# ppwwyyxx/speaker-recognition

Hardware: AMD Instinct MI355X
Metric: frames/sec scored (MFCC+GMM) (higher is better)
Workload: dtype f32

## Files before the change

speaker-recognition_amd/csrc/abi.cpp:

```cpp
#include "../../include/pygmm_hip.h"

#include "batch.hpp"
#include "common.hpp"
#include "fork_proxy.hpp"
#include "gmm_full.hpp"
#include "gmm_model.hpp"
#include "mfcc.hpp"
#include "mfcc_plan.hpp"
#include "score.hpp"
#include "silence_plan.hpp"
#include "topc_plan.hpp"
#include "bw_plan.hpp"
#include "jfa_plan.hpp"
#include "map_plan.hpp"

#include <algorithm>
#include <cmath>
#include <cstring>
#include <fstream>
#include <limits>
#include <sstream>

namespace sr {
void burn_reference_rand(int count);
// ... 1132 lines not shown
    ltsd_compute(*pcm, winsize, order, noise_amp, ltsd_out, win_offsets_out);
    return 0;
    SR_CATCH(-1)
}

int sr_set_option(const char *key, long value) {
    SR_TRY
    if (!key) fail("null key");
    const std::string k(key);
    if (k == "score_frames_per_lane") {
        if (value != 0 && value != 1 && value != 2 && value != 4) fail("frames per lane must be 0/1/2/4");
        score_options().frames_per_lane = (int)value;
    } else if (k == "score_model_groups") {
        score_options().model_groups = (int)value;
    } else if (k == "score_packed") {
        score_options().packed = (int)value;
    } else if (k == "score_engine") {
        if (value < 0 || value > 6 || value == 2)
            fail("score_engine must be 0 (auto), 1 (vector ALU), 3 (split-bf16 matrix cores), 4 (split-bf16, shared-sigma form), "
                 "5 (split-fp16 matrix cores) or 6 (split-fp16, shared-sigma form); 2 was the fp32 matrix-core engine, removed in round 5 "
                 "(never selected: 1.45-1.8x slower than split-bf16 at the same accuracy)");
        score_options().engine = (int)value;
    } else if (k == "score_h2s_shape") {
        if (value < 0 || value > 5)
            fail("score_h2s_shape must be 0 (automatic), 1 (4-wave workgroups), 2 (12-wave workgroups), 3 (12 waves, image loop pipelined inside the wave), "
                 "4 (4 waves on one tile, the block's models split between them) or 5 (as 3, on the flat image where 3 takes the compact one)");
        score_options().h2s_shape = (int)value;
    } else if (k == "flush_list_cap") {
        if (value < 0) fail("flush_list_cap must be >= 0");
        score_options().flush_list_cap = (int)value;
    } else if (k == "score_h2s_pack_tails") {
        if (value != 0 && value != 1) fail("score_h2s_pack_tails must be 0 or 1");
        score_options().h2s_pack_tails = (int)value;
    } else if (k == "score_h2s_force_exc") {
        score_options().h2s_force_exc = value != 0;
    } else if (k == "score_split_shape") {
        if (value != 0 && value != 1 && value != 8 && value != 12 && value != 16)
            fail("score_split_shape must be 0 (automatic), 1 (4-wave workgroups) or 8 / 12 / 16 (waves of the wide, pipelined form)");
        score_options().split_shape = (int)value;
    } else if (k == "score_mfma_ft") {
        if (value < 0 || value > 4) fail("score_mfma_ft must be 0..4");
        score_options().mfma_ft = (int)value;
    } else if (k == "flush_order") {
        if (value != 1 && value != 2)
            fail("flush_order must be 2 (partial products as the reference DSO's compiler forms them: even / odd dimensions) or "
                 "1 (the source's order, gmm.cc:192-195)");
        flush_order_option() = (int)value;
    } else if (k == "kmeans_assign_engine") {
        if (value != 0 && value != 1) fail("kmeans_assign_engine must be 0 (fast full search, exact pass for what it cannot decide) or 1 (exact pass only)");
// ... 219 lines not shown
```

speaker-recognition_amd/csrc/gmm_score_h2_shared.hip:

```cpp
#include "lse.hpp"
#include "score.hpp"
#include "wave_ops.hpp"

#include <algorithm>
#include <cstdint>
#include <type_traits>

namespace sr {

typedef float f32x16 __attribute__((ext_vector_type(16)));
typedef _Float16 f16x8 __attribute__((ext_vector_type(8)));
typedef unsigned u32x4 __attribute__((ext_vector_type(4)));

constexpr int H2S_ROUNDS_PER_LAUNCH = 12;
constexpr float H2S_SUM_LO = 7.8886090522101181e-31f;
constexpr float H2S_SUM_HI = 1.2676506002282294e+30f;
constexpr float H2S_LOG2E = 1.4426950408889634f;

template <int KN, int KM, int COLS>
__device__ __forceinline__ void h2s_chain_regs(f32x16 (&acc)[COLS], const f32x16 (&init)[COLS], const uint4 (&fr)[KM],
                                               const f16x8 (&b)[COLS][KN]) {
#pragma unroll
    for (int ks = 0; ks < KN; ks++)
#pragma unroll
// ... 518 lines not shown
    else if constexpr (NX == 1) H2P_SLOT_ASM(H, R, NA_, 1);     \
    else if constexpr (NX == 2) H2P_SLOT_ASM(H, R, NA_, 2);     \
    else if constexpr (NX == 3) H2P_SLOT_ASM(H, R, NA_, 3);     \
    else H2P_SLOT_ASM(H, R, NA_, 4);
#define H2P_SLOT_NA(H, R)                                \
    if constexpr (NA == 0) { H2P_SLOT_NX(H, R, 0) }      \
    else if constexpr (NA == 1) { H2P_SLOT_NX(H, R, 1) } \
    else if constexpr (NA == 2) { H2P_SLOT_NX(H, R, 2) } \
    else if constexpr (NA == 3) { H2P_SLOT_NX(H, R, 3) } \
    else { H2P_SLOT_NX(H, R, 4) }
template <int HEAD, bool READ, int NA, int NX, int W, int O>
__device__ __forceinline__ void h2p_slot(f32x16 &cur, u32x4 &fu, float &s, float &e0, float &e1, float &e2, float &e3, const f16x8 &b, const f32x16 &c,
                                         unsigned at, float p0, float p1, float p2, float p3) {
    static_assert(NA <= 4 && NX <= 4, "at most four exps per slot");
    if constexpr (HEAD == 0) {
        if constexpr (READ) { H2P_SLOT_NA(0, 1) } else { H2P_SLOT_NA(0, 0) }
    } else if constexpr (HEAD == 1) {
        if constexpr (READ) { H2P_SLOT_NA(1, 1) } else { H2P_SLOT_NA(1, 0) }
    } else {
        if constexpr (READ) { H2P_SLOT_NA(2, 1) } else { H2P_SLOT_NA(2, 0) }
    }
}

template <int KQF, int KLF, bool CPT = false>
__global__ __launch_bounds__(12 * 64, 3)
void gmm_score_h2p_kernel(const H2sArgs a) {
    constexpr int SB = SHARED_SB, WAVES = 12, G = 4, NB = 2, DMA_AT = KLF / 2;
    constexpr int KM = KQF > KLF ? KQF : KLF;
    static_assert(KQF <= KLF, "the linear half is never the shorter one");
    static_assert(!CPT || (KQF == H2C_KLF && KLF == H2C_KLF), "the compact order is built for the <8,8> chains");
    static_assert(!CPT || h2c_map_ok(H2C_MAP), "compact order");
    constexpr int NF = CPT ? H2C_MAP.nf : KM;
    constexpr int NBQ = CPT ? H2C_MAP.nb : KQF, NBL = CPT ? H2C_MAP.nb : KLF;
    constexpr int IMG_U4 = NF * 64;
    constexpr int STAGE_U4 = G * IMG_U4;
    constexpr int N_IMG = 1 + SB;
    constexpr int N_STAGES = N_IMG / G;
    static_assert(N_IMG % G == 0 && N_STAGES >= 1, "stages tile the images of a mixture tile");
    extern __shared__ uint4 h2s_bq_lds[];
    __shared__ uint4 ring[NB * STAGE_U4];

    const int tid = threadIdx.x;
    const int lane = tid & 63;
    const int wave = __builtin_amdgcn_readfirstlane(tid >> 6);
    const int col = lane & 31;
    const int hh = lane >> 5;

    constexpr int N_PIECES = STAGE_U4 / 64;
    constexpr int P_LO = N_PIECES / WAVES, P_HI = (N_PIECES + WAVES - 1) / WAVES, N_HI = N_PIECES % WAVES;
    auto stage_load = [&](int slot, const uint4 *src) {
#pragma unroll
        for (int i = 0; i < P_HI; i++) {
            const int piece = i * WAVES + wave;
            if (piece < N_PIECES)
                __builtin_amdgcn_global_load_lds(
                    (const __attribute__((address_space(1))) void *)(src + piece * 64 + lane),
                    (__attribute__((address_space(3))) void *)(ring + slot * STAGE_U4 + piece * 64), 16, 0, 0);
        }
    };
    auto wait_stages = [&](int keep) {
        if (keep <= 0 || P_HI == 0) {
// ... 26 lines not shown
        tile = a.tiles[has ? tids[0] : 0];
#pragma unroll
        for (int p = 1; p < 4; p++)
            if (p < n_seg && col >= first_col[p]) {
                my_col = col - first_col[p];
                tile = a.tiles[tids[p]];
            }
    }
    const bool valid = has && my_col < tile.count;
    const int64_t row = tile.start + (valid ? my_col : 0);
    {
        f16x8 bq[NBQ];
        h2s_build_b<NBQ>(bq, a.X + row * a.dim, a.center, a.scale, a.q_desc, hh, true, zmax);
#pragma unroll
        for (int ks = 0; ks < NBQ; ks++) h2s_bq_lds[(wave * NBQ + ks) * 64 + lane] = __builtin_bit_cast(uint4, bq[ks]);
    }
    h2s_build_b<NBL>(bl, a.X + row * a.dim, a.center, a.scale, a.l_desc, hh, false, zmax);
    const float off = a.ref_ll[row] * H2S_LOG2E;
    if (zmax >= 255.0f) atomicOr(a.oor_flag, 1);
    const float safe_ll2 = a.clamp ? fmaxf(LSE_MINLOG2 + LSE_NEAR + a.log2_k, a.band_hi * H2S_LOG2E + 1.0f) : -3.0e38f;
    const f32x16 zero1 = {0, 0, 0, 0, 0, 0, 0, 0, 0, 0, 0, 0, 0, 0, 0, 0};
    const unsigned ring_lane = (unsigned)(uintptr_t)(__attribute__((address_space(3))) void *)ring + (unsigned)lane * 16u;

    for (int blk = blk_begin; blk < blk_end; blk++) {
        const SharedBlock sb = a.blocks[blk];
        const uint4 *stream = a.params + sb.offset_u4;
        float ssum[SB + 1];
#pragma unroll
        for (int si = 0; si <= SB; si++) ssum[si] = 0.0f;
        const int n_st = (1 + sb.n_models + G - 1) / G;
        const int n_stage_total = a.n_mix_tiles * n_st;
        int ld_tile = 0, ld_st = 0;
        auto stage_load_next = [&](int slot) {
            stage_load(slot, stream + (size_t)ld_tile * (N_IMG * IMG_U4) + (size_t)ld_st * STAGE_U4);
            if (++ld_st == n_st) {
                ld_st = 0;
                ld_tile++;
            }
        };
        u32x4 fr[NF];
        auto frag_read = [&](auto U, unsigned at) {
            constexpr int u = decltype(U)::value;
            u32x4 &dst = fr[u];
            asm volatile("ds_read_b128 %0, %1 offset:%2" : "=v"(dst) : "v"(at), "n"(u * 1024));
        };

        asm volatile("s_waitcnt lgkmcnt(0)" ::: "memory");
        barrier();
        stage_load_next(0);
        if (n_stage_total > 1) stage_load_next(1);
        if (NB > 2 && n_stage_total > 2) stage_load_next(2);
        wait_stages(n_stage_total > NB - 1 ? NB - 1 : n_stage_total - 1);
        barrier();
        h2p_for<0, (CPT ? NF : KQF)>([&](auto U) { frag_read(U, ring_lane); });

        f32x16 acc[2];
        acc[0] = zero1;
#pragma unroll
        for (int r = 0; r < 16; r++) acc[1][r] = -1.0e30f;
        int S = 0, slot_cur = 0, slot_nxt = 1;
        static_assert(NB == 2 || NB == 3, "ring of two or three stages");
        f32x16 qacc = zero1;
        float e[16] = {0.0f, 0.0f, 0.0f, 0.0f};
        for (int t = 0; t < a.n_mix_tiles; t++) {
            h2p_for<0, N_IMG>([&](auto IMG) {
                constexpr int img = decltype(IMG)::value;
                constexpr int gi = img % G;
                constexpr int kn = img == 0 ? KQF : KLF;
                constexpr int kn_next = img + 1 == N_IMG ? KQF : KLF;
                constexpr bool carry = img != 1;
                constexpr int prev_model = img == 0 ? SB : img - 2;
                if (img / G >= n_st) return;
                if constexpr (gi == G - 1) {
                    wait_stages(NB > 2 && S + 2 < n_stage_total ? 1 : 0);
                    barrier();
                    if constexpr (DMA_AT == 0)
                        if (S + NB < n_stage_total) stage_load_next(slot_cur);
                }
                const unsigned next_at = ring_lane + (unsigned)((gi == G - 1 ? slot_nxt * STAGE_U4 : slot_cur * STAGE_U4 + (gi + 1) * IMG_U4) * 16);
                f32x16 &cur = img == 0 ? qacc : acc[img & 1];
                const f32x16 &prev = acc[(img & 1) ^ 1];
                constexpr int BW = KQF < 4 ? KQF : 4;
                f16x8 bqt[BW];
                auto bq_load = [&](int ks) { return __builtin_bit_cast(f16x8, h2s_bq_lds[(wave * NBQ + ks) * 64 + lane]); };
                if constexpr (img == 0) {
                    if constexpr (CPT) {
                        h2p_for<0, BW>([&](auto KS) { bqt[decltype(KS)::value] = bq_load(H2C_MAP.b_of[decltype(KS)::value]); });
                    } else {
#pragma unroll
                        for (int ks = 0; ks < BW; ks++) bqt[ks] = bq_load(ks);
                    }
                }
                constexpr bool ONE_ASM = kn >= 5;
                static_assert(!CPT || ONE_ASM, "the compact order is written for the one-statement slots");
                constexpr int sum_model = carry ? prev_model : 0;
                if constexpr (ONE_ASM) {
                    h2p_for<0, kn>([&](auto U) {
                        constexpr int u = decltype(U)::value;
                        if constexpr (gi == G - 1 && DMA_AT != 0 && u == DMA_AT)
                            if (S + NB < n_stage_total) stage_load_next(slot_cur);
                        constexpr int fa = CPT ? H2C_MAP.a_of[u] : u, bi = CPT ? H2C_MAP.b_of[u] : u;
                        constexpr bool rd = CPT ? H2C_MAP.a_last[fa] == u : (u < kn_next);
                        constexpr int younger = CPT ? h2c_younger(H2C_MAP, u) : (kn - 1 - u) + (u < kn_next ? u : kn_next);
                        static_assert(younger <= 15, "lgkmcnt is a 4-bit field");
                        constexpr int e0 = carry ? h2p_cum(kn, u - 2) : 0, e1 = carry ? h2p_cum(kn, u - 1) : 0, e2 = carry ? h2p_cum(kn, u) : 0;
                        constexpr int NA = e1 - e0, NX = e2 - e1;
                        const float p0 = prev[e1 < 16 ? e1 : 15], p1 = prev[e1 + 1 < 16 ? e1 + 1 : 15], p2 = prev[e1 + 2 < 16 ? e1 + 2 : 15],
                                    p3 = prev[e1 + 3 < 16 ? e1 + 3 : 15];
                        if constexpr (img == 0)
                        {
                            h2p_slot<u == 0 ? 0 : 2, rd, NA, NX, younger, fa * 1024>(cur, fr[fa], ssum[sum_model], e[0], e[1], e[2], e[3], bqt[u % BW],
                                                                                     qacc, next_at, p0, p1, p2, p3);
                            if constexpr (u + BW < KQF) bqt[u % BW] = bq_load(CPT ? H2C_MAP.b_of[u + BW] : u + BW);
                        }
                        else
                            h2p_slot<u == 0 ? 1 : 2, rd, NA, NX, younger, fa * 1024>(cur, fr[fa], ssum[sum_model], e[0], e[1], e[2], e[3], bl[bi], qacc,
                                                                                     next_at, p0, p1, p2, p3);
                        __builtin_amdgcn_sched_barrier(0);
                    });
                } else {
                    h2p_for<0, kn>([&](auto U) {
                        constexpr int u = decltype(U)::value;
                        if constexpr (gi == G - 1 && DMA_AT != 0 && u == DMA_AT)
                            if (S + NB < n_stage_total) stage_load_next(slot_cur);
                        constexpr int younger = (kn - 1 - u) + (u < kn_next ? u : kn_next);
                        u32x4 &fu = fr[u];
                        asm volatile("s_waitcnt lgkmcnt(%1)" : "+v"(fu) : "n"(younger));
                        if constexpr (img == 0)
                            cur = __builtin_amdgcn_mfma_f32_32x32x16_f16(__builtin_bit_cast(f16x8, fr[u]), bqt[u % BW], u == 0 ? zero1 : cur, 0, 0, 0);
                        else
                            cur = __builtin_amdgcn_mfma_f32_32x32x16_f16(__builtin_bit_cast(f16x8, fr[u]), bl[u], u == 0 ? qacc : cur, 0, 0, 0);
                        f32x16 &cpin = cur;
                        asm volatile("" : "+v"(cpin));
                        if constexpr (u < kn_next) frag_read(U, next_at);
                        if constexpr (carry) {
                            constexpr int e0 = h2p_cum(kn, u - 2), e1 = h2p_cum(kn, u - 1), e2 = h2p_cum(kn, u);
                            h2p_for<e0, e1>([&](auto R) {
                                float &sv = ssum[prev_model];
                                const float ev = e[decltype(R)::value - e0];
                                asm volatile("v_add_f32 %0, %0, %1" : "+v"(sv) : "v"(ev));
                            });
                            h2p_for<e1, e2>([&](auto R) {
                                float &ev = e[decltype(R)::value - e1];
                                const float pv = prev[decltype(R)::value];
                                asm volatile("v_exp_f32 %0, %1" : "=v"(ev) : "v"(pv));
                            });
                        }
                        __builtin_amdgcn_sched_barrier(0);
                    });
                }
                if constexpr (!CPT) h2p_for<kn, kn_next>([&](auto U) { frag_read(U, next_at); });
                if constexpr (carry) {
                    constexpr int e0 = h2p_cum(kn, kn - 2), e1 = h2p_cum(kn, kn - 1);
                    if constexpr (kn <= 1) {
#pragma unroll
                        for (int r = 0; r < 16; r++) ssum[prev_model] += __builtin_amdgcn_exp2f(prev[r]);
                    } else {
                        asm volatile("s_nop 0");
                        h2p_for<e0, e1>([&](auto R) {
                            float &sv = ssum[prev_model];
                            const float ev = e[decltype(R)::value - e0];
                            asm volatile("v_add_f32 %0, %0, %1" : "+v"(sv) : "v"(ev));
                        });
                    }
                }
                if constexpr (img == 0) {
                    asm volatile("s_nop 12");
                    h2p_for<0, 16>([&](auto R) {
                        float x = qacc[decltype(R)::value];
                        asm volatile("v_sub_f32 %0, %0, %1" : "+v"(x) : "v"(off));
                        qacc[decltype(R)::value] = x;
                    });
                    asm volatile("s_nop 1");
                }
                __builtin_amdgcn_sched_barrier(0);
                if constexpr (gi == G - 1) {
                    S++;
                    slot_cur = slot_nxt;
                    slot_nxt = slot_nxt == NB - 1 ? 0 : slot_nxt + 1;
                }
            });
        }
        asm volatile("s_nop 12");
#pragma unroll
        for (int r = 0; r < 16; r++) ssum[SB] += __builtin_amdgcn_exp2f(acc[(N_IMG - 1) & 1][r]);
        float fin[SB];
        const int last_model = n_st * G - 2;
#pragma unroll
        for (int si = 0; si < SB; si++) fin[si] = ssum[si] + (si == last_model ? ssum[SB] : 0.0f);
        {
            int tids[4], first_col[4], n_seg;
            h2p_unit(a, unit, tids, first_col, n_seg);
            if (n_seg == 1) h2s_close_block(a, sb, blk, fin, off, valid, has, tids[0], row, lane, hh, safe_ll2);
            else h2s_close_block_packed(a, sb, blk, fin, off, valid, has, tids, first_col, n_seg, row, lane, hh, safe_ll2);
        }
    }
    asm volatile("s_waitcnt lgkmcnt(0)" ::: "memory");
}

__device__ __forceinline__ int *h2s_plan_starts(const H2sArgs &a, int blk) {
    return reinterpret_cast<int *>(a.exc_list + (size_t)a.n_blocks * a.n_tiles) + (size_t)blk * (a.n_tiles + 1);
}

constexpr int H2S_PLAN_INLINE_MAX_TILES = 1024;
__device__ __forceinline__ int h2s_plan_block(const H2sArgs &a, int blk, int lane) {
    const int count = min(a.exc_count[blk], a.n_tiles);
    int *starts = h2s_plan_starts(a, blk);
    const int2 *list = a.exc_list + (size_t)blk * a.n_tiles;
    int n_items = 0, fill = 32;
    for (int base = 0; base < count; base += 64) {
        const int pop = base + lane < count ? __builtin_popcount((unsigned)list[base + lane].y) : 0;
        const int n = min(64, count - base);
        for (int i = 0; i < n; i++) {
            const int p = __builtin_amdgcn_readlane(pop, i);
            if (fill + p > 32) {
                if (lane == 0) starts[n_items] = base + i;
                n_items++;
// ... 163 lines not shown
        for (int o = 32; o > 0; o >>= 1) max_pop = max(max_pop, __shfl_xor(max_pop, o));
        const unsigned own_cols = pop >= 32 ? 0xffffffffu : ((1u << pop) - 1u);
#pragma unroll
        for (int si = 0; si < SB; si++) {
            const float ll = lse_close2(mx[si], ssum[si], other_half(mx[si]), other_half(ssum[si]), a.clamp);
            const bool live = has && valid && hh == 0 && si < sb.n_models;
            const double v = live ? (double)ll : 0.0;
            if (live && a.frame_ll) a.frame_ll[(int64_t)(sb.first_model + si) * a.n_frames + row] = ll;
            const unsigned hot_cols = (unsigned)__builtin_amdgcn_ballot_w64(live && ll < a.band_hi);
            double sum = 0.0;
            for (int j = 0; j < max_pop; j++) {
                const double t = shfl_f64(v, min(excl + j, 31));
                if (j < pop) sum += t;
            }
            if (has && lane < n_ent && si < sb.n_models) {
                double *p = a.partial + (int64_t)ent.x * a.n_models + sb.first_model + si;
                *p = ((hot_cols >> excl) & own_cols) != 0 ? SR_FLUSH_POISON : *p + sum;
            }
            __builtin_amdgcn_sched_barrier(0);
        }
    }
}

template <int KQF, int KLF, int COLS, int WAVES, bool PIN = false, bool MS = false, bool CPT = false>
static int launch_h2s(const H2sLaunch &l) {
    static_assert(!CPT || PIN, "the compact image is the pipelined kernel's");
    constexpr int MQ = CPT ? H2C_KLF : KQF, ML = CPT ? H2C_KLF : KLF;
    constexpr bool BQ_LDS = h2s_bq_in_lds(KQF, KLF, WAVES);
    H2sArgs a;
    a.X = l.X;
    a.tiles = l.tiles;
    a.params = reinterpret_cast<const uint4 *>(l.params);
    a.blocks = l.blocks;
    a.group_block_begin = l.group_block_begin;
    a.center = l.center;
    a.scale = l.scale;
    a.q_desc = l.q_desc;
    a.l_desc = l.l_desc;
    a.ref_ll = l.ref_ll;
    a.partial = l.partial;
    a.frame_ll = l.frame_ll;
    a.oor_flag = l.oor_flag;
    a.exc_list = reinterpret_cast<int2 *>(l.exc_list);
    a.exc_count = l.exc_count;
    a.n_blocks = l.n_blocks;
    a.n_frames = l.n_frames;
    a.dim = l.dim;
    a.n_models = l.n_models;
    a.n_mix_tiles = l.n_mix_tiles;
// ... 17 lines not shown
    a.n_units = PIN ? (l.n_work + H2P_ROUND_ITEMS - 1) / H2P_ROUND_ITEMS * H2P_ROUND_ITEMS : l.n_tiles;
    static_assert(!PIN || H2P_ROUND_ITEMS % TILES_WG == 0, "a workgroup's work items never straddle the table's padding");
    int wg_per_launch = WAVES > 4 ? std::max(8, (n_wg + 7) / 8 * 8)
                        : std::max(8, (H2S_ROUNDS_PER_LAUNCH * resident / std::max(1, l.n_groups)) / 8 * 8);
    int n_launches = 0;
    for (int base = 0; base < n_wg; base += wg_per_launch) {
        n_launches++;
        a.tile_base = base * TILES_WG;
        const int n = std::min(wg_per_launch, n_wg - base);
        const int per_xcd = ((l.n_groups + 7) / 8) * n;
        const bool xcd_groups = MS && KLF <= H2M_MAX_KLF && l.n_groups > 1 && n == n_wg && per_xcd <= 2 * (ctx().n_cu / 8);
        dim3 grid(xcd_groups ? (unsigned)(8 * ((l.n_groups + 7) / 8) * n) : (unsigned)((int64_t)l.n_groups * ((n + 7) / 8) * 8));
        a.rows8 = (n + 7) / 8;
        a.n_wg = n;
        a.group_major = xcd_groups ? 2 : l.n_groups > 1;
        constexpr bool M_DIRECT = MS && KLF <= H2M_MAX_KLF;
        constexpr size_t dyn = CPT      ? (size_t)WAVES * H2C_MAP.nb * 64 * sizeof(uint4)
                               : M_DIRECT ? 0
                                          : (BQ_LDS ? (size_t)WAVES * KQF * 64 * sizeof(uint4) : 0) + (MS ? sizeof(uint4) : 0);
        if constexpr (dyn > 0) {
            static bool attr_set[MAX_DEVICES] = {};
            if (!attr_set[ctx().device]) {
                if constexpr (PIN)
                    SR_HIP(hipFuncSetAttribute(reinterpret_cast<const void *>(&gmm_score_h2p_kernel<MQ, ML, CPT>),
                                               hipFuncAttributeMaxDynamicSharedMemorySize, (int)dyn));
                else
                    SR_HIP(hipFuncSetAttribute(reinterpret_cast<const void *>(&gmm_score_h2s_kernel<KQF, KLF, COLS, WAVES, MS>),
                                               hipFuncAttributeMaxDynamicSharedMemorySize, (int)dyn));
                attr_set[ctx().device] = true;
            }
        }
        if constexpr (PIN)
            hipLaunchKernelGGL((gmm_score_h2p_kernel<MQ, ML, CPT>), grid, dim3(WAVES * 64), dyn, ctx().stream, a);
        else if constexpr (M_DIRECT)
            hipLaunchKernelGGL((gmm_score_h2m_kernel<KQF, KLF>), grid, dim3(WAVES * 64), 0, ctx().stream, a);
        else
            hipLaunchKernelGGL((gmm_score_h2s_kernel<KQF, KLF, COLS, WAVES, MS>), grid, dim3(WAVES * 64), dyn, ctx().stream, a);
    }
    a.tile_base = 0;
    if constexpr (CPT) {
        a.params = reinterpret_cast<const uint4 *>(l.params);
        a.blocks = l.blocks;
        a.q_desc = l.q_desc;
        a.l_desc = l.l_desc;
    }
    if (!a.plan_inline) hipLaunchKernelGGL(h2s_plan_kernel, dim3((unsigned)l.n_blocks), dim3(64), 0, ctx().stream, a);
    const int gy = std::max(1, (2 * ctx().n_cu) / std::max(1, l.n_blocks));
    hipLaunchKernelGGL((gmm_score_h2s_online_kernel<KQF, KLF>), dim3((unsigned)(l.n_blocks * gy)), dim3(256), 0, ctx().stream, a);
    return n_launches;
}

int launch_score_h2_shared(const H2sLaunch &l, int KQF, int KLF) {
#define SR_H2S_CASE(Q, L)                                       \
    if (KQF == Q && KLF == L) {                                 \
        if constexpr (L == H2C_KLF)                             \
            if (l.shape == 2 && l.c_params) return launch_h2s<Q, L, 1, 12, true, false, true>(l); \
        if constexpr (h2p_fits(Q, L))                           \
            if (l.shape == 2) return launch_h2s<Q, L, 1, 12, true>(l); \
        if (l.shape == 3) return launch_h2s<Q, L, 1, 4, false, true>(l); \
        if (l.shape >= 1) return launch_h2s<Q, L, 1, 12>(l);    \
        return launch_h2s<Q, L, 1, 4>(l);                       \
    }
    SR_H2S_CASE(1, 1) SR_H2S_CASE(1, 2) SR_H2S_CASE(2, 2) SR_H2S_CASE(3, 3) SR_H2S_CASE(3, 4) SR_H2S_CASE(4, 4)
    SR_H2S_CASE(4, 5) SR_H2S_CASE(5, 5) SR_H2S_CASE(6, 6) SR_H2S_CASE(6, 7) SR_H2S_CASE(7, 7)
    SR_H2S_CASE(7, 8) SR_H2S_CASE(8, 8) SR_H2S_CASE(9, 9) SR_H2S_CASE(9, 10)
#undef SR_H2S_CASE
    fail("no split-fp16 shared-sigma scoring kernel for %d + %d contraction steps", KQF, KLF);
}

}
```

speaker-recognition_amd/csrc/gmm_score_host.cpp:

```cpp
#include "score.hpp"

#include <algorithm>
#include <cmath>
#include <cstring>

namespace sr {

struct LastKernel {
    char name[256] = "";
};
#define g_last_kernel (per_device<LastKernel>().name)
const char *last_score_kernel() { return g_last_kernel; }

struct PassCounters {
    int *oor_p() { return buf.p; }
    int *flush_count_p() { return buf.p + 1; }
    int *exc_count_p() { return buf.p + 4; }
    int *base() { return buf.p; }
    void begin(size_t n, bool delivering) {
        buf.ensure(n);
        if (!(delivering && clean_p == buf.p && clean_n >= n)) {
            SR_HIP(hipMemsetAsync(buf.p, 0, n * sizeof(int), ctx().stream));
        } else if (score_options().verify_clean_counters) {
            std::vector<int> h(n);
// ... 83 lines not shown
    s.d_h2s_params.upload(h.params.data(), h.params.size());
    s.d_h2s_blocks.upload(h.blocks.data(), h.blocks.size());
    s.d_h2s_center.upload(h.center.data(), h.center.size());
    s.d_h2s_scale.upload(h.scale.data(), h.scale.size());
    s.d_h2s_qdesc.upload(h.q_desc.data(), h.q_desc.size());
    s.d_h2s_ldesc.upload(h.l_desc.data(), h.l_desc.size());
    s.d_h2s_ref_params.upload(h.ref.params.data(), h.ref.params.size());
    s.d_h2s_ref_chunks.upload(h.ref.chunks.data(), h.ref.chunks.size());
    const int gcb[2] = {0, (int)h.ref.chunks.size()};
    s.d_h2s_ref_gcb.upload(gcb, 2);
    s.d_h2s_ref_center.upload(h.ref.center.data(), h.ref.center.size());
    s.d_h2s_ref_scale.upload(h.ref.scale.data(), h.ref.scale.size());
    sync_stream();
}

static bool ensure_h2c_layout(SRModelSet &s) {
    if (s.h2c_state != 0) return s.h2c_state > 0;
    const PackedH2Shared &h = s.h2s;
    if (!h2c_built(s.host.dim, h.klf)) {
        s.h2c_state = -1;
        return false;
    }
    const PackedH2Compact c = pack_h2_compact(h, s.host.dim);
    s.d_h2c_params.upload(c.params.data(), c.params.size());
    s.d_h2c_blocks.upload(c.blocks.data(), c.blocks.size());
    s.d_h2c_qdesc.upload(c.q_desc.data(), c.q_desc.size());
    s.d_h2c_ldesc.upload(c.l_desc.data(), c.l_desc.size());
    sync_stream();
    s.h2c_nk = c.nk;
    s.h2c_state = 1;
    return true;
}

static void ensure_h2_layout(SRModelSet &s) {
    if (s.d_h2_params.p) return;
    s.d_h2_params.upload(s.h2.params.data(), s.h2.params.size());
    s.d_h2_chunks.upload(s.h2.chunks.data(), s.h2.chunks.size());
    s.d_h2_center.upload(s.h2.center.data(), s.h2.center.size());
    s.d_h2_scale.upload(s.h2.scale.data(), s.h2.scale.size());
    sync_stream();
}

void ensure_bx3_layout(SRModelSet &s) {
    if (s.d_bx3_params.p && !s.bx3_stale) return;
    s.bx3_stale = false;
    s.d_bx3_params.upload(s.bx3.params.data(), s.bx3.params.size());
    s.d_bx3_chunks.upload(s.bx3.chunks.data(), s.bx3.chunks.size());
// ... 78 lines not shown
    a.params = set.d_h2s_params.p;
    a.blocks = set.d_h2s_blocks.p;
    a.group_block_begin = c.d_gcb;
    a.center = set.d_h2s_center.p;
    a.scale = set.d_h2s_scale.p;
    a.q_desc = set.d_h2s_qdesc.p;
    a.l_desc = set.d_h2s_ldesc.p;
    a.ref_ll = w.ref_ll.p;
    a.oor_flag = w.counters.oor_p();
    a.exc_list = w.exc_list.p;
    a.exc_count = w.counters.exc_count_p();
    a.n_blocks = n_blocks;
    a.n_mix_tiles = h.n_tiles;
    a.log2_k = (float)std::log2((double)h.n_tiles * MT);
    a.force_exc = opt.h2s_force_exc;
    a.shape = h2s_shape;
    bool compact = false;
    if (h2s_shape == 2) {
        ensure_work_table(tt, opt.h2s_pack_tails != 0);
        a.tiles = tt.d_tiles_work.p;
        a.n_work = tt.n_work;
        compact = opt.h2s_shape != 5 && ensure_h2c_layout(set);
        if (compact) {
            a.c_params = set.d_h2c_params.p;
            a.c_blocks = set.d_h2c_blocks.p;
            a.c_q_desc = set.d_h2c_qdesc.p;
            a.c_l_desc = set.d_h2c_ldesc.p;
        }
    }
    snprintf(g_last_kernel, sizeof(LastKernel::name),
             "%s<%d,%d,%s>%s (shared sigma: quadratic half once per %d models; split-fp16 MFMA, "
             "3 products as one contraction; reference-offset log-sum-exp)", h2s_shape == 2 ? "gmm_score_h2p_kernel" : (h2s_shape == 3 && h2s_msplit_direct(h.klf)) ? "gmm_score_h2m_kernel" : "gmm_score_h2s_kernel",
             compact ? set.h2c_nk : h.kqf, compact ? set.h2c_nk : h.klf,
             h2s_shape == 2 ? "waves=12, pipelined in the wave" : h2s_shape == 1 ? "waves=12" : h2s_shape == 3 ? "waves=4 on one tile, models split" : "waves=4",
             compact ? "/compact" : "", SHARED_SB);
    ScopedKernelTimer t(T_SCORE);
    const int n_launches = launch_score_h2_shared(a, h.kqf, h.klf);
    const size_t len = strlen(g_last_kernel);
    snprintf(g_last_kernel + len, sizeof(LastKernel::name) - len, " [%d launches per pass]", n_launches);
}

static void launch_shared_bf16(SRModelSet &set, const PassArgs &c) {
    ensure_shared_layout(set);
    SharedLaunch a = common_args<SharedLaunch>(c);
    a.params = set.d_shared_params.p;
    a.blocks = set.d_shared_blocks.p;
    a.group_block_begin = c.d_gcb;
    a.center = set.d_shared_center.p;
    a.n_mix_tiles = set.shared.n_tiles;
    snprintf(g_last_kernel, sizeof(LastKernel::name),
             "gmm_score_bx3_shared_kernel<%d,%d> (shared sigma: quadratic half once per %d models; split-bf16 MFMA)",
             set.shared.kq, set.shared.kl, SHARED_SB);
    ScopedKernelTimer t(T_SCORE);
    launch_score_bx3_shared(a, set.shared.kq, set.shared.kl);
}

static void launch_split(SRModelSet &set, const ScorePlan &plan, const PassArgs &c) {
    const bool use_h2 = plan.engine == Engine::SPLIT_F16;
// ... 397 lines not shown
```

speaker-recognition_amd/csrc/score.hpp:

```cpp
#pragma once

#include "batch.hpp"
#include "gmm_model.hpp"
#include "score_plan.hpp"

namespace sr {

constexpr int SCORE_NO_FLUSH = 0x400;
constexpr int SCORE_HOST_DELIVER = 0x800;
constexpr size_t HOST_DELIVER_MAX_BYTES = (size_t)64 << 10;
constexpr size_t HOST_DELIVER_MAX_UTTS = 256;
inline bool host_deliverable(size_t n_utt, size_t n_models) {
    return n_utt > 0 && n_utt <= HOST_DELIVER_MAX_UTTS && n_utt * n_models * sizeof(double) + n_utt * sizeof(int) <= HOST_DELIVER_MAX_BYTES;
}
struct DeliverHeader {
    int oor, n_flush;
    unsigned seq;
    int pad;
};

struct ScoreArgs {
    const float *X;
    const TileDesc *tiles;
    const float4 *params;
// ... 55 lines not shown
    const float *X;
    const TileDesc *tiles;
    const uint16_t *params;
    const SharedBlock *blocks;
    const int *group_block_begin;
    const float *center, *scale;
    const uint16_t *q_desc, *l_desc;
    const float *ref_ll;
    double *partial;
    float *frame_ll;
    int *oor_flag;
    int n_work = 0;
    int *exc_list;
    int *exc_count;
    int n_blocks;
    int64_t n_frames;
    int dim, n_models, n_mix_tiles, clamp, n_groups, n_tiles;
    float log2_k;
    int force_exc;
    int shape = 0;
    const uint16_t *c_params = nullptr;
    const SharedBlock *c_blocks = nullptr;
    const uint16_t *c_q_desc = nullptr, *c_l_desc = nullptr;
    float band_hi = -__builtin_inff();
};
int launch_score_h2_shared(const H2sLaunch &a, int KQF, int KLF);
void launch_score_split(const MfmaLaunch &a, int scheme, int KS, int FT);
bool launch_score_splitp(const MfmaLaunch &a, int scheme, int KS, int waves, int chunks_per_model);
const char *last_score_kernel();

struct ScoreResult {
    const double *d_sums = nullptr;
    const int *d_argmax = nullptr;
    const float *d_frame_ll = nullptr;
    const int *d_oor = nullptr;
    const int *d_flush_count = nullptr;
    const int2 *d_flush_list = nullptr;
    int flush_cap = 0;
    const TileTable *tiles = nullptr;
    const volatile DeliverHeader *h_deliver = nullptr;
    unsigned deliver_seq = 0;
};

struct OpenSetRule {
    int bg;
    double threshold;
// ... 88 lines not shown
```

speaker-recognition_amd/csrc/score_plan.cpp:

```cpp
#include "score_plan.hpp"

#include <algorithm>
#include <cmath>

namespace sr {

ScoreOptions &score_options() {
    static ScoreOptions o;
    return o;
}

static int auto_frames_per_lane(int64_t n_rows, int n_utt, int dp) {
    const int fmax = dp <= 40 ? 4 : dp <= 64 ? 2 : 1;
    if (n_utt == 0) return 1;
    const double mean_len = (double)n_rows / n_utt;
    for (int f = fmax; f > 1; f >>= 1) {
        const double tile = 256.0 * f;
        const double tiles = std::ceil(mean_len / tile);
        if (mean_len / (tiles * tile) >= 0.80) return f;
    }
    return 1;
}

static Engine precise_engine(const SRModelSet &set) {
// ... 30 lines not shown
        case 0: return auto_engine(set, precise);
        default: return Engine::VECTOR;
    }
}

ScorePlan plan_score(const SRModelSet &set, int64_t n_rows, int n_utt, const ScoreOptions &opt, int flags, int n_cu) {
    const int S = set.host.n_models;
    const int DP = set.host.dp;
    ScorePlan p;
    p.engine = pick_engine(set, opt.engine, (flags & SCORE_PRECISE) != 0);
    const PackedSplit &split = p.engine == Engine::SPLIT_F16 ? set.h2 : set.bx3;
    int F = opt.frames_per_lane ? opt.frames_per_lane : auto_frames_per_lane(n_rows, n_utt, DP);
    if (DP > 40 && F > 2) F = 2;
    if (DP > 64) F = 1;
    if (!opt.frames_per_lane)
        while (F > 1 && ((n_rows + 256 * F - 1) / (256 * F)) * (int64_t)std::max(1, S) < 2 * (int64_t)n_cu) F >>= 1;
    p.F = F;
    if (p.split()) p.FT = opt.mfma_ft ? std::min(opt.mfma_ft, split_max_ft(split.ks)) : 1;
    const int64_t n32 = (n_rows + 31) / 32 + n_utt;
    if (p.engine == Engine::SHARED_F16) {
        const bool wide = n32 >= 64 + n_utt;
        const int64_t ms_wgs = n32 * (int64_t)set.h2s.blocks.size();
        const bool tiny = ms_wgs <= (int64_t)n_cu * (h2s_msplit_direct(set.h2s.klf) ? 2 : 1);
        p.h2s_shape = opt.h2s_shape == 5 ? H2S_PIPELINED_SHAPE : opt.h2s_shape ? opt.h2s_shape - 1 : (tiny ? H2S_MSPLIT_SHAPE : wide ? H2S_PIPELINED_SHAPE : 0);
        if (p.h2s_shape == H2S_PIPELINED_SHAPE && !h2p_fits(set.h2s.kqf, set.h2s.klf)) p.h2s_shape = H2S_WIDE_SHAPE;
    }
    if (p.engine == Engine::SPLIT_F16 && p.FT == 1 && opt.split_shape != 1) {
        const std::vector<int> &mcb = split.model_chunk_begin;
        p.split_cpm = S > 0 ? mcb[1] - mcb[0] : 0;
        for (int s = 1; s < S; s++)
            if (mcb[s + 1] - mcb[s] != p.split_cpm) p.split_cpm = 0;
        if (p.split_cpm > 0) {
            const int w = splitp_waves_f16x2(split.ks, opt.split_shape ? opt.split_shape : 8);
            if (w > 0 && (opt.split_shape || (split.ks >= 5 && (int64_t)S * p.split_cpm >= 32 &&
                                              (n32 / w) * (int64_t)std::min(S, 16) >= (int64_t)6 * n_cu * splitp_resident_per_cu(w))))
                p.splitp_w = w;
        }
    }
    const bool mat = p.engine != Engine::VECTOR;
    p.tile_frames = (p.engine == Engine::SHARED_F16 || p.split()) ? 32 : mat ? 128 * p.FT : 256 * F;
    p.per_tile = mat ? 1 : 4;
    p.writes_oor = p.engine == Engine::SHARED_F16 || p.engine == Engine::SPLIT_F16;
    return p;
}

std::vector<int> plan_groups(const SRModelSet &set, const ScorePlan &p, int n_tiles, const ScoreOptions &opt, int n_cu) {
    const bool use_h2s = p.engine == Engine::SHARED_F16, use_shared = p.engine == Engine::SHARED_BF16, use_split = p.split();
// ... 161 lines not shown
```

speaker-recognition_amd/csrc/score_shapes.hpp:

```cpp
#pragma once

#include <initializer_list>

#if defined(__HIPCC__)
#define SR_HD __host__ __device__
#else
#define SR_HD
#endif

namespace sr {

SR_HD constexpr int h2s_waves_per_eu(int kqf, int klf, int cols, int waves, bool ms = false) {
    (void)kqf; (void)klf; (void)cols; (void)ms;
    return waves > 4 ? waves / 4 : 2;
}
constexpr int H2M_MAX_KLF = 9;
SR_HD constexpr bool h2p_fits(int kqf, int klf) { return klf >= 2 && kqf <= klf && (2 * 4 * klf + 12 * kqf) * 1024 <= 160 * 1024; }

constexpr int H2C_MAX_STEPS = 16;
struct H2cMap {
    int h = 0, nk = 0, nf = 0, nb = 0;
    int a_of[H2C_MAX_STEPS] = {}, b_of[H2C_MAX_STEPS] = {};
    int a_last[H2C_MAX_STEPS] = {}, b_last[H2C_MAX_STEPS] = {};
    int a_half[H2C_MAX_STEPS][2] = {}, b_half[H2C_MAX_STEPS][2] = {};
// ... 43 lines not shown
    if (m.nk > H2C_MAX_STEPS || m.nf > m.nk || m.nb > m.nk || m.nk != h2c_steps(m.h)) return false;
    for (int f = 0; f < m.nf; f++) {
        bool used = false;
        for (int s = 0; s < m.nk; s++) used = used || m.a_of[s] == f;
        if (!used || (f > 0 && m.a_last[f] <= m.a_last[f - 1])) return false;
    }
    for (int r = 0; r < m.nb; r++) {
        bool used = false;
        for (int s = 0; s < m.nk; s++) used = used || m.b_of[s] == r;
        if (!used) return false;
    }
    for (int s = 0; s < m.nk; s++)
        if (m.a_of[s] < 0 || m.a_of[s] >= m.nf || m.b_of[s] < 0 || m.b_of[s] >= m.nb || h2c_younger(m, s) > 15) return false;
    return true;
}
constexpr int H2C_KLF = 8, H2C_H = 5;
constexpr H2cMap H2C_MAP = h2c_map(H2C_H);
static_assert(h2c_map_ok(h2c_map(H2C_H)) && h2c_map(H2C_H).nk == H2C_KLF && h2c_map(H2C_H).nf == 6 && h2c_map(H2C_H).nb == 6, "the compact order of the <8,8> chains");
static_assert(h2c_map_ok(h2c_map(4)) && h2c_map_ok(h2c_map(3)) && h2c_map_ok(h2c_map(6)) && h2c_map_ok(h2c_map(1)), "even and odd part lengths");
SR_HD constexpr bool h2c_built(int dim, int klf) { return klf == H2C_KLF && h2c_applies(dim, klf) && h2c_half_steps(dim) == H2C_H; }
SR_HD constexpr int h2c_lds_bytes(int h) { return (2 * 4 * h2c_map(h).nf + 12 * h2c_map(h).nb) * 1024; }
static_assert(h2c_lds_bytes(H2C_H) <= 160 * 1024 && (4 * h2c_map(H2C_H).nf) % 12 == 0, "the compact ring fits a CU; a stage is a whole number of pieces per wave");

constexpr int h2s_resident_per_cu(int kqf, int klf, int shape) { return (shape == 0 || shape == 3) ? h2s_waves_per_eu(kqf, klf, 1, 4, shape == 3) : 1; }
constexpr int h2s_tiles_per_wg(int shape) { return shape == 0 ? 4 : shape == 3 ? 1 : 12; }
constexpr bool h2s_msplit_direct(int klf) { return klf <= H2M_MAX_KLF; }

constexpr int split_max_ft(int ks) { return ks <= 6 ? 2 : 1; }

SR_HD constexpr int splitp_stage_chunks(int ks, int parts, int waves) { return waves > 8 && ks * parts <= 10 ? 4 : 2; }
SR_HD constexpr int splitp_lds_bytes(int ks, int parts, int waves) {
    return 3 * splitp_stage_chunks(ks, parts, waves) * ks * parts * 1024 + waves * 16 * 33 * 4;
}
SR_HD constexpr bool splitp_fits(int ks, int parts, int waves) {
    if (waves != 12 && ks * parts > 10) return false;
    return splitp_lds_bytes(ks, parts, waves) <= (160 * 1024 - 512) / (waves > 8 ? 1 : 2);
}
constexpr int splitp_resident_per_cu(int waves) { return waves > 8 ? 1 : 2; }
inline int splitp_waves_f16x2(int ks, int want) {
    const int parts = 2;
    if (ks < 2 || ks > 8) return 0;
    for (int w : {want, 16, 12, 8})
        if ((w == 16 || w == 12 || w == 8) && splitp_fits(ks, parts, w)) return w;
    return 0;
}

// ... 2 lines not shown
```

Baseline: 39.18 million.

## Pair consecutive model blocks in pipelined compact scoring kernel sharing one quadratic half

Adds a PAIR variant of the pipelined compact h2p kernel that processes two consecutive 15-model blocks in one pass, forming the shared quadratic image once per pair instead of once per block. This cuts the number of images streamed and multiplied per group (e.g. 216 down to 210 for 201 models) and the per-block pipeline restart overhead. The pairing is made the default for the compact path (shape 6 restores one quadratic half per block), and the device parameter buffer is zero-padded so the second block's stream offset stays in bounds. It adds extra per-lane sums and register copies between tiles, which may raise register pressure.

```diff
diff --git a/speaker-recognition_amd/csrc/abi.cpp b/speaker-recognition_amd/csrc/abi.cpp
--- a/speaker-recognition_amd/csrc/abi.cpp
+++ b/speaker-recognition_amd/csrc/abi.cpp
@@ -1178,9 +1178,10 @@
                  "(never selected: 1.45-1.8x slower than split-bf16 at the same accuracy)");
         score_options().engine = (int)value;
     } else if (k == "score_h2s_shape") {
-        if (value < 0 || value > 5)
+        if (value < 0 || value > 6)
             fail("score_h2s_shape must be 0 (automatic), 1 (4-wave workgroups), 2 (12-wave workgroups), 3 (12 waves, image loop pipelined inside the wave), "
-                 "4 (4 waves on one tile, the block's models split between them) or 5 (as 3, on the flat image where 3 takes the compact one)");
+                 "4 (4 waves on one tile, the block's models split between them), 5 (as 3, on the flat image where 3 takes the compact one) "
+                 "or 6 (as 3, one quadratic half per block where 3 forms one per two blocks)");
         score_options().h2s_shape = (int)value;
     } else if (k == "flush_list_cap") {
         if (value < 0) fail("flush_list_cap must be >= 0");
diff --git a/speaker-recognition_amd/csrc/gmm_score_h2_shared.hip b/speaker-recognition_amd/csrc/gmm_score_h2_shared.hip
--- a/speaker-recognition_amd/csrc/gmm_score_h2_shared.hip
+++ b/speaker-recognition_amd/csrc/gmm_score_h2_shared.hip
@@ -564,7 +564,7 @@
     }
 }
 
-template <int KQF, int KLF, bool CPT = false>
+template <int KQF, int KLF, bool CPT = false, bool PAIR = false>
 __global__ __launch_bounds__(12 * 64, 3)
 void gmm_score_h2p_kernel(const H2sArgs a) {
     constexpr int SB = SHARED_SB, WAVES = 12, G = 4, NB = 2, DMA_AT = KLF / 2;
@@ -572,13 +572,15 @@
     static_assert(KQF <= KLF, "the linear half is never the shorter one");
     static_assert(!CPT || (KQF == H2C_KLF && KLF == H2C_KLF), "the compact order is built for the <8,8> chains");
     static_assert(!CPT || h2c_map_ok(H2C_MAP), "compact order");
+    static_assert(!PAIR || (CPT && SB == H2Q_SB && G == H2Q_G), "pairs of blocks: the compact form, blocks of 15, stages of four");
     constexpr int NF = CPT ? H2C_MAP.nf : KM;
     constexpr int NBQ = CPT ? H2C_MAP.nb : KQF, NBL = CPT ? H2C_MAP.nb : KLF;
     constexpr int IMG_U4 = NF * 64;
     constexpr int STAGE_U4 = G * IMG_U4;
-    constexpr int N_IMG = 1 + SB;
-    constexpr int N_STAGES = N_IMG / G;
-    static_assert(N_IMG % G == 0 && N_STAGES >= 1, "stages tile the images of a mixture tile");
+    constexpr int N_IMG_T = 1 + SB;
+    constexpr int N_IMG = PAIR ? 1 + 2 * SB : 1 + SB;
+    constexpr int N_STAGES = N_IMG_T / G;
+    static_assert(N_IMG_T % G == 0 && N_STAGES >= 1, "stages tile the images of a mixture tile");
     extern __shared__ uint4 h2s_bq_lds[];
     __shared__ uint4 ring[NB * STAGE_U4];
 
@@ -651,17 +653,32 @@
     const f32x16 zero1 = {0, 0, 0, 0, 0, 0, 0, 0, 0, 0, 0, 0, 0, 0, 0, 0};
     const unsigned ring_lane = (unsigned)(uintptr_t)(__attribute__((address_space(3))) void *)ring + (unsigned)lane * 16u;
 
-    for (int blk = blk_begin; blk < blk_end; blk++) {
+    int n_blk = 1;
+    for (int blk = blk_begin; blk < blk_end; blk += n_blk) {
         const SharedBlock sb = a.blocks[blk];
         const uint4 *stream = a.params + sb.offset_u4;
+        const uint4 *stream2 = stream;
+        int m2 = 0;
+        if constexpr (PAIR) {
+            if (blk + 1 < blk_end && h2q_pairs(SB, sb.n_models, 1)) {
+                const SharedBlock sb2 = a.blocks[blk + 1];
+                m2 = sb2.n_models;
+                stream2 = a.params + sb2.offset_u4 + (size_t)h2q_stage_image(SB, G, N_STAGES) * IMG_U4 - (size_t)N_STAGES * STAGE_U4;
+            }
+            n_blk = m2 > 0 ? 2 : 1;
+        }
         float ssum[SB + 1];
+        float ssum2[PAIR ? SB : 1];
 #pragma unroll
         for (int si = 0; si <= SB; si++) ssum[si] = 0.0f;
-        const int n_st = (1 + sb.n_models + G - 1) / G;
+#pragma unroll
+        for (int si = 0; si < (PAIR ? SB : 1); si++) ssum2[si] = 0.0f;
+        const int n_st = h2q_stages(G, sb.n_models, m2);
+        const bool last_even = PAIR && n_st * G > N_IMG;
         const int n_stage_total = a.n_mix_tiles * n_st;
         int ld_tile = 0, ld_st = 0;
         auto stage_load_next = [&](int slot) {
-            stage_load(slot, stream + (size_t)ld_tile * (N_IMG * IMG_U4) + (size_t)ld_st * STAGE_U4);
+            stage_load(slot, (PAIR && ld_st >= N_STAGES ? stream2 : stream) + (size_t)ld_tile * (N_IMG_T * IMG_U4) + (size_t)ld_st * STAGE_U4);
             if (++ld_st == n_st) {
                 ld_st = 0;
                 ld_tile++;
@@ -687,28 +704,30 @@
         acc[0] = zero1;
 #pragma unroll
         for (int r = 0; r < 16; r++) acc[1][r] = -1.0e30f;
+        if constexpr (PAIR) acc[0] = acc[1];
         int S = 0, slot_cur = 0, slot_nxt = 1;
         static_assert(NB == 2 || NB == 3, "ring of two or three stages");
         f32x16 qacc = zero1;
         float e[16] = {0.0f, 0.0f, 0.0f, 0.0f};
         for (int t = 0; t < a.n_mix_tiles; t++) {
-            h2p_for<0, N_IMG>([&](auto IMG) {
+            auto image = [&](auto IMG, auto PSEL) {
                 constexpr int img = decltype(IMG)::value;
                 constexpr int gi = img % G;
+                constexpr bool los = gi == G - 1 || img == N_IMG - 1;
                 constexpr int kn = img == 0 ? KQF : KLF;
                 constexpr int kn_next = img + 1 == N_IMG ? KQF : KLF;
                 constexpr bool carry = img != 1;
                 constexpr int prev_model = img == 0 ? SB : img - 2;
                 if (img / G >= n_st) return;
-                if constexpr (gi == G - 1) {
+                if constexpr (los) {
                     wait_stages(NB > 2 && S + 2 < n_stage_total ? 1 : 0);
                     barrier();
                     if constexpr (DMA_AT == 0)
                         if (S + NB < n_stage_total) stage_load_next(slot_cur);
                 }
-                const unsigned next_at = ring_lane + (unsigned)((gi == G - 1 ? slot_nxt * STAGE_U4 : slot_cur * STAGE_U4 + (gi + 1) * IMG_U4) * 16);
+                const unsigned next_at = ring_lane + (unsigned)((los ? slot_nxt * STAGE_U4 : slot_cur * STAGE_U4 + (gi + 1) * IMG_U4) * 16);
                 f32x16 &cur = img == 0 ? qacc : acc[img & 1];
-                const f32x16 &prev = acc[(img & 1) ^ 1];
+                const f32x16 &prev = acc[decltype(PSEL)::value];
                 constexpr int BW = KQF < 4 ? KQF : 4;
                 f16x8 bqt[BW];
                 auto bq_load = [&](int ks) { return __builtin_bit_cast(f16x8, h2s_bq_lds[(wave * NBQ + ks) * 64 + lane]); };
@@ -723,10 +742,12 @@
                 constexpr bool ONE_ASM = kn >= 5;
                 static_assert(!CPT || ONE_ASM, "the compact order is written for the one-statement slots");
                 constexpr int sum_model = carry ? prev_model : 0;
+                constexpr bool second = PAIR && carry && img != 0 && img - 2 >= SB;
+                float &sum_ref = second ? ssum2[second ? img - 2 - SB : 0] : ssum[second ? 0 : sum_model];
                 if constexpr (ONE_ASM) {
                     h2p_for<0, kn>([&](auto U) {
                         constexpr int u = decltype(U)::value;
-                        if constexpr (gi == G - 1 && DMA_AT != 0 && u == DMA_AT)
+                        if constexpr (los && DMA_AT != 0 && u == DMA_AT)
                             if (S + NB < n_stage_total) stage_load_next(slot_cur);
                         constexpr int fa = CPT ? H2C_MAP.a_of[u] : u, bi = CPT ? H2C_MAP.b_of[u] : u;
                         constexpr bool rd = CPT ? H2C_MAP.a_last[fa] == u : (u < kn_next);
@@ -738,19 +759,19 @@
                                     p3 = prev[e1 + 3 < 16 ? e1 + 3 : 15];
                         if constexpr (img == 0)
                         {
-                            h2p_slot<u == 0 ? 0 : 2, rd, NA, NX, younger, fa * 1024>(cur, fr[fa], ssum[sum_model], e[0], e[1], e[2], e[3], bqt[u % BW],
+                            h2p_slot<u == 0 ? 0 : 2, rd, NA, NX, younger, fa * 1024>(cur, fr[fa], sum_ref, e[0], e[1], e[2], e[3], bqt[u % BW],
                                                                                      qacc, next_at, p0, p1, p2, p3);
                             if constexpr (u + BW < KQF) bqt[u % BW] = bq_load(CPT ? H2C_MAP.b_of[u + BW] : u + BW);
                         }
                         else
-                            h2p_slot<u == 0 ? 1 : 2, rd, NA, NX, younger, fa * 1024>(cur, fr[fa], ssum[sum_model], e[0], e[1], e[2], e[3], bl[bi], qacc,
+                            h2p_slot<u == 0 ? 1 : 2, rd, NA, NX, younger, fa * 1024>(cur, fr[fa], sum_ref, e[0], e[1], e[2], e[3], bl[bi], qacc,
                                                                                      next_at, p0, p1, p2, p3);
                         __builtin_amdgcn_sched_barrier(0);
                     });
                 } else {
                     h2p_for<0, kn>([&](auto U) {
                         constexpr int u = decltype(U)::value;
-                        if constexpr (gi == G - 1 && DMA_AT != 0 && u == DMA_AT)
+                        if constexpr (los && DMA_AT != 0 && u == DMA_AT)
                             if (S + NB < n_stage_total) stage_load_next(slot_cur);
                         constexpr int younger = (kn - 1 - u) + (u < kn_next ? u : kn_next);
                         u32x4 &fu = fr[u];
@@ -787,7 +808,7 @@
                     } else {
                         asm volatile("s_nop 0");
                         h2p_for<e0, e1>([&](auto R) {
-                            float &sv = ssum[prev_model];
+                            float &sv = sum_ref;
                             const float ev = e[decltype(R)::value - e0];
                             asm volatile("v_add_f32 %0, %0, %1" : "+v"(sv) : "v"(ev));
                         });
@@ -803,25 +824,46 @@
                     asm volatile("s_nop 1");
                 }
                 __builtin_amdgcn_sched_barrier(0);
-                if constexpr (gi == G - 1) {
+                if constexpr (los) {
                     S++;
                     slot_cur = slot_nxt;
                     slot_nxt = slot_nxt == NB - 1 ? 0 : slot_nxt + 1;
                 }
+            };
+            h2p_for<0, N_IMG>([&](auto IMG) {
+                constexpr int img = decltype(IMG)::value;
+                image(IMG, std::integral_constant<int, PAIR && img == 0 ? 0 : (img & 1) ^ 1>{});
             });
+            if constexpr (PAIR) {
+                if (!last_even) {
+                    f32x16 &from = acc[1];
+                    asm volatile("s_nop 12" : "+v"(from));
+                    h2p_for<0, 16>([&](auto R) {
+                        float x;
+                        const float y = acc[1][decltype(R)::value];
+                        asm volatile("v_mov_b32 %0, %1" : "=v"(x) : "v"(y));
+                        acc[0][decltype(R)::value] = x;
+                    });
+                }
+                __builtin_amdgcn_sched_barrier(0);
+            }
         }
         asm volatile("s_nop 12");
 #pragma unroll
-        for (int r = 0; r < 16; r++) ssum[SB] += __builtin_amdgcn_exp2f(acc[(N_IMG - 1) & 1][r]);
-        float fin[SB];
-        const int last_model = n_st * G - 2;
-#pragma unroll
-        for (int si = 0; si < SB; si++) fin[si] = ssum[si] + (si == last_model ? ssum[SB] : 0.0f);
-        {
+        for (int r = 0; r < 16; r++) ssum[SB] += __builtin_amdgcn_exp2f(acc[PAIR ? 0 : (N_IMG - 1) & 1][r]);
+        const int last_model = (last_even ? N_IMG : n_st * G) - 2;
+        for (int half = 0; half < (PAIR ? n_blk : 1); half++) {
+            const SharedBlock sbh = PAIR ? a.blocks[blk + half] : sb;
+            float fin[SB];
+#pragma unroll
+            for (int si = 0; si < SB; si++) {
+                const float own = PAIR && half ? ssum2[PAIR ? si : 0] : ssum[si];
+                fin[si] = own + (half * SB + si == last_model ? ssum[SB] : 0.0f);
+            }
             int tids[4], first_col[4], n_seg;
             h2p_unit(a, unit, tids, first_col, n_seg);
-            if (n_seg == 1) h2s_close_block(a, sb, blk, fin, off, valid, has, tids[0], row, lane, hh, safe_ll2);
-            else h2s_close_block_packed(a, sb, blk, fin, off, valid, has, tids, first_col, n_seg, row, lane, hh, safe_ll2);
+            if (n_seg == 1) h2s_close_block(a, sbh, blk + half, fin, off, valid, has, tids[0], row, lane, hh, safe_ll2);
+            else h2s_close_block_packed(a, sbh, blk + half, fin, off, valid, has, tids, first_col, n_seg, row, lane, hh, safe_ll2);
         }
     }
     asm volatile("s_waitcnt lgkmcnt(0)" ::: "memory");
@@ -1031,9 +1073,10 @@
     }
 }
 
-template <int KQF, int KLF, int COLS, int WAVES, bool PIN = false, bool MS = false, bool CPT = false>
+template <int KQF, int KLF, int COLS, int WAVES, bool PIN = false, bool MS = false, bool CPT = false, bool PAIR = false>
 static int launch_h2s(const H2sLaunch &l) {
     static_assert(!CPT || PIN, "the compact image is the pipelined kernel's");
+    static_assert(!PAIR || CPT, "blocks go in pairs on the compact image only");
     constexpr int MQ = CPT ? H2C_KLF : KQF, ML = CPT ? H2C_KLF : KLF;
     constexpr bool BQ_LDS = h2s_bq_in_lds(KQF, KLF, WAVES);
     H2sArgs a;
@@ -1097,7 +1140,7 @@
             static bool attr_set[MAX_DEVICES] = {};
             if (!attr_set[ctx().device]) {
                 if constexpr (PIN)
-                    SR_HIP(hipFuncSetAttribute(reinterpret_cast<const void *>(&gmm_score_h2p_kernel<MQ, ML, CPT>),
+                    SR_HIP(hipFuncSetAttribute(reinterpret_cast<const void *>(&gmm_score_h2p_kernel<MQ, ML, CPT, PAIR>),
                                                hipFuncAttributeMaxDynamicSharedMemorySize, (int)dyn));
                 else
                     SR_HIP(hipFuncSetAttribute(reinterpret_cast<const void *>(&gmm_score_h2s_kernel<KQF, KLF, COLS, WAVES, MS>),
@@ -1106,7 +1149,7 @@
             }
         }
         if constexpr (PIN)
-            hipLaunchKernelGGL((gmm_score_h2p_kernel<MQ, ML, CPT>), grid, dim3(WAVES * 64), dyn, ctx().stream, a);
+            hipLaunchKernelGGL((gmm_score_h2p_kernel<MQ, ML, CPT, PAIR>), grid, dim3(WAVES * 64), dyn, ctx().stream, a);
         else if constexpr (M_DIRECT)
             hipLaunchKernelGGL((gmm_score_h2m_kernel<KQF, KLF>), grid, dim3(WAVES * 64), 0, ctx().stream, a);
         else
@@ -1129,7 +1172,7 @@
 #define SR_H2S_CASE(Q, L)                                       \
     if (KQF == Q && KLF == L) {                                 \
         if constexpr (L == H2C_KLF)                             \
-            if (l.shape == 2 && l.c_params) return launch_h2s<Q, L, 1, 12, true, false, true>(l); \
+            if (l.shape == 2 && l.c_params) return l.pair ? launch_h2s<Q, L, 1, 12, true, false, true, true>(l) : launch_h2s<Q, L, 1, 12, true, false, true>(l); \
         if constexpr (h2p_fits(Q, L))                           \
             if (l.shape == 2) return launch_h2s<Q, L, 1, 12, true>(l); \
         if (l.shape == 3) return launch_h2s<Q, L, 1, 4, false, true>(l); \
diff --git a/speaker-recognition_amd/csrc/gmm_score_host.cpp b/speaker-recognition_amd/csrc/gmm_score_host.cpp
--- a/speaker-recognition_amd/csrc/gmm_score_host.cpp
+++ b/speaker-recognition_amd/csrc/gmm_score_host.cpp
@@ -129,7 +129,10 @@
         return false;
     }
     const PackedH2Compact c = pack_h2_compact(h, s.host.dim);
+    const size_t pad_u16 = (size_t)c.nf * 64 * 8;
+    s.d_h2c_params.ensure(c.params.size() + pad_u16);
     s.d_h2c_params.upload(c.params.data(), c.params.size());
+    SR_HIP(hipMemsetAsync(s.d_h2c_params.p + c.params.size(), 0, pad_u16 * sizeof(uint16_t), ctx().stream));
     s.d_h2c_blocks.upload(c.blocks.data(), c.blocks.size());
     s.d_h2c_qdesc.upload(c.q_desc.data(), c.q_desc.size());
     s.d_h2c_ldesc.upload(c.l_desc.data(), c.l_desc.size());
@@ -254,6 +257,7 @@
         a.n_work = tt.n_work;
         compact = opt.h2s_shape != 5 && ensure_h2c_layout(set);
         if (compact) {
+            a.pair = opt.h2s_shape != 6;
             a.c_params = set.d_h2c_params.p;
             a.c_blocks = set.d_h2c_blocks.p;
             a.c_q_desc = set.d_h2c_qdesc.p;
@@ -265,7 +269,7 @@
              "3 products as one contraction; reference-offset log-sum-exp)", h2s_shape == 2 ? "gmm_score_h2p_kernel" : (h2s_shape == 3 && h2s_msplit_direct(h.klf)) ? "gmm_score_h2m_kernel" : "gmm_score_h2s_kernel",
              compact ? set.h2c_nk : h.kqf, compact ? set.h2c_nk : h.klf,
              h2s_shape == 2 ? "waves=12, pipelined in the wave" : h2s_shape == 1 ? "waves=12" : h2s_shape == 3 ? "waves=4 on one tile, models split" : "waves=4",
-             compact ? "/compact" : "", SHARED_SB);
+             compact ? "/compact" : "", a.pair ? 2 * SHARED_SB : SHARED_SB);
     ScopedKernelTimer t(T_SCORE);
     const int n_launches = launch_score_h2_shared(a, h.kqf, h.klf);
     const size_t len = strlen(g_last_kernel);
diff --git a/speaker-recognition_amd/csrc/score.hpp b/speaker-recognition_amd/csrc/score.hpp
--- a/speaker-recognition_amd/csrc/score.hpp
+++ b/speaker-recognition_amd/csrc/score.hpp
@@ -101,6 +101,7 @@
     const uint16_t *c_params = nullptr;
     const SharedBlock *c_blocks = nullptr;
     const uint16_t *c_q_desc = nullptr, *c_l_desc = nullptr;
+    bool pair = false;
     float band_hi = -__builtin_inff();
 };
 int launch_score_h2_shared(const H2sLaunch &a, int KQF, int KLF);
diff --git a/speaker-recognition_amd/csrc/score_plan.cpp b/speaker-recognition_amd/csrc/score_plan.cpp
--- a/speaker-recognition_amd/csrc/score_plan.cpp
+++ b/speaker-recognition_amd/csrc/score_plan.cpp
@@ -76,7 +76,7 @@
         const bool wide = n32 >= 64 + n_utt;
         const int64_t ms_wgs = n32 * (int64_t)set.h2s.blocks.size();
         const bool tiny = ms_wgs <= (int64_t)n_cu * (h2s_msplit_direct(set.h2s.klf) ? 2 : 1);
-        p.h2s_shape = opt.h2s_shape == 5 ? H2S_PIPELINED_SHAPE : opt.h2s_shape ? opt.h2s_shape - 1 : (tiny ? H2S_MSPLIT_SHAPE : wide ? H2S_PIPELINED_SHAPE : 0);
+        p.h2s_shape = (opt.h2s_shape == 5 || opt.h2s_shape == 6) ? H2S_PIPELINED_SHAPE : opt.h2s_shape ? opt.h2s_shape - 1 : (tiny ? H2S_MSPLIT_SHAPE : wide ? H2S_PIPELINED_SHAPE : 0);
         if (p.h2s_shape == H2S_PIPELINED_SHAPE && !h2p_fits(set.h2s.kqf, set.h2s.klf)) p.h2s_shape = H2S_WIDE_SHAPE;
     }
     if (p.engine == Engine::SPLIT_F16 && p.FT == 1 && opt.split_shape != 1) {
diff --git a/speaker-recognition_amd/csrc/score_shapes.hpp b/speaker-recognition_amd/csrc/score_shapes.hpp
--- a/speaker-recognition_amd/csrc/score_shapes.hpp
+++ b/speaker-recognition_amd/csrc/score_shapes.hpp
@@ -89,6 +89,36 @@
 SR_HD constexpr int h2c_lds_bytes(int h) { return (2 * 4 * h2c_map(h).nf + 12 * h2c_map(h).nb) * 1024; }
 static_assert(h2c_lds_bytes(H2C_H) <= 160 * 1024 && (4 * h2c_map(H2C_H).nf) % 12 == 0, "the compact ring fits a CU; a stage is a whole number of pieces per wave");
 
+constexpr int H2Q_SB = 15, H2Q_G = 4;
+SR_HD constexpr bool h2q_pairs(int sb, int m1, int m2) { return m2 > 0 && m1 == sb; }
+SR_HD constexpr int h2q_stages(int g, int m1, int m2) { return (1 + m1 + m2 + g - 1) / g; }
+SR_HD constexpr int h2q_images(int sb, int g, int m1, int m2) {
+    return h2q_stages(g, m1, m2) * g < 1 + 2 * sb ? h2q_stages(g, m1, m2) * g : 1 + 2 * sb;
+}
+SR_HD constexpr int h2q_last_image(int sb, int g, int m1, int m2) { return h2q_images(sb, g, m1, m2) - 1; }
+SR_HD constexpr int h2q_last_parity(int sb, int g, int m1, int m2) { return h2q_last_image(sb, g, m1, m2) & 1; }
+SR_HD constexpr int h2q_last_model(int sb, int g, int m1, int m2) { return h2q_last_image(sb, g, m1, m2) - 1; }
+SR_HD constexpr int h2q_stage_block(int sb, int g, int s) { return s * g < 1 + sb ? 0 : 1; }
+SR_HD constexpr int h2q_stage_image(int sb, int g, int s) { return s * g < 1 + sb ? s * g : s * g - sb; }
+static_assert((1 + H2Q_SB) % H2Q_G == 0 && h2q_stages(H2Q_G, H2Q_SB, H2Q_SB) == 8 && h2q_images(H2Q_SB, H2Q_G, H2Q_SB, H2Q_SB) == 31 &&
+              h2q_last_parity(H2Q_SB, H2Q_G, H2Q_SB, H2Q_SB) == 0 && h2q_last_parity(H2Q_SB, H2Q_G, H2Q_SB, 6) == 1 &&
+              h2q_stage_image(H2Q_SB, H2Q_G, 4) == 1 && h2q_stage_image(H2Q_SB, H2Q_G, 7) == 13, "a full pair: 31 images, the last an even one");
+SR_HD constexpr int h2q_group_images(int sb, int g, int n_models, bool paired) {
+    int n = 0, left = n_models;
+    while (left > 0) {
+        const int m1 = left < sb ? left : sb;
+        left -= m1;
+        int m2 = 0;
+        if (paired && left > 0 && m1 == sb) {
+            m2 = left < sb ? left : sb;
+            left -= m2;
+        }
+        n += h2q_images(sb, g, m1, m2);
+    }
+    return n;
+}
+static_assert(h2q_group_images(H2Q_SB, H2Q_G, 201, false) == 216 && h2q_group_images(H2Q_SB, H2Q_G, 201, true) == 210, "BASELINE configs[2]: 201 models");
+
 constexpr int h2s_resident_per_cu(int kqf, int klf, int shape) { return (shape == 0 || shape == 3) ? h2s_waves_per_eu(kqf, klf, 1, 4, shape == 3) : 1; }
 constexpr int h2s_tiles_per_wg(int shape) { return shape == 0 ? 4 : shape == 3 ? 1 : 12; }
 constexpr bool h2s_msplit_direct(int klf) { return klf <= H2M_MAX_KLF; }
```

Result: faster. 40.10 million, median of 6 (+2.3%).
